# anulum/scpn-fusion-core

Measured on NVIDIA B200. Metric: converged_equilibria_per_s, higher is better.
Workload: dtype f64

## Files before the change

### scpn_fusion_core_b200/csrc/gsb_picard.cu

```cuda
#include "gsb_internal.cuh"
#include "gsb_resident.cuh"

#include <algorithm>
#include <cstdlib>

constexpr int kPT = 32;
constexpr int kTW = 8;
constexpr int kRW = 4;
constexpr int kSadChunk = 4096;
constexpr int kSadChunksMax = 64;

struct PicardState {
  int *active, *status, *iter, *cur, *best, *nxt, *xsel, *seed_active;
  double *diff_best, *gs_best, *gs_last, *diff_last, *scale;
  double *axbnd;
  double *topo;
};

struct Bufs {
  double *p[3];
};

struct gsb_picard_ws {
  int cap = 0;
// ... 957 lines not shown
  if (ir >= nr || iz >= nz) return;
  const size_t n = (size_t)nz * nr;
  double gz, gr;
  grad_point(psi + b * n, nz, nr, iz, ir, gg, gz, gr);
  const double rs = fmax(rrow[ir], 1e-6);
  const double inv = __ddiv_rn(1.0, rs);
  br[b * n + (size_t)iz * nr + ir] = dmul(-inv, gz);
  bz[b * n + (size_t)iz * nr + ir] = dmul(inv, gr);
}


struct PicardResArgs {
  double *psi;
  const double *bc;
  const double *ip;
  const double *prof_dev;
  double *jphi;
  double *summary;
  double *hist, *gs_hist;
  double *ws_psi;
  double *ws_src;
  const double *seedJ, *cf, *mr, *rrow;
  const int *rowmask;
  double seed_sum_drdz;
  int batch, max_iter, seed, saddle, need_gs, external;
  double tol, gs_tol, alpha, oma, omega;
  double dr, dz, dr2, dz2, four_drdz;
  GradGeom gg;
  ProfileDev prof;
  int scratch_off;
  int tplane_off;
  const int *order;
  const int *n_order;
};

__device__ __forceinline__ double pl(int xo, int nz, int hw, int iz, int ir) {
  return res_pool[xo + split_index(nz, hw, iz, ir)];
}

__device__ __forceinline__ void grad_planes(int xo, int nz, int nr, int hw, int iz, int ir, const GradGeom &gg,
                                            double &gz, double &gr) {
  const double c = pl(xo, nz, hw, iz, ir);
  if (iz == 0)
    gz = ddiv_y(dsub(pl(xo, nz, hw, 1, ir), c), gg.dz, gg.inv_dz);
  else if (iz == nz - 1)
    gz = ddiv_y(dsub(c, pl(xo, nz, hw, iz - 1, ir)), gg.dz, gg.inv_dz);
  else
    gz = ddiv_y(dsub(pl(xo, nz, hw, iz + 1, ir), pl(xo, nz, hw, iz - 1, ir)), gg.two_dz, gg.inv_two_dz);
  if (ir == 0)
    gr = ddiv_y(dsub(pl(xo, nz, hw, iz, 1), c), gg.dr, gg.inv_dr);
  else if (ir == nr - 1)
    gr = ddiv_y(dsub(c, pl(xo, nz, hw, iz, ir - 1)), gg.dr, gg.inv_dr);
  else
    gr = ddiv_y(dsub(pl(xo, nz, hw, iz, ir + 1), pl(xo, nz, hw, iz, ir - 1)), gg.two_dr, gg.inv_two_dr);
}

__device__ __forceinline__ double grad_mag(const GradGeom &gg, double c, double up, double down, double left,
                                           double right, bool z_lo, bool z_hi, bool r_lo, bool r_hi) {
  double gz, gr;
  if (z_lo)
    gz = ddiv_yf(dsub(up, c), gg.dz, gg.inv_dz);
  else if (z_hi)
    gz = ddiv_yf(dsub(c, down), gg.dz, gg.inv_dz);
  else
    gz = ddiv_yf(dsub(up, down), gg.two_dz, gg.inv_two_dz);
  if (r_lo)
// ... 11 lines not shown
  MtanhK mkp, mkf;
};
__device__ __forceinline__ double jraw_point(const JrawK &K, double v, double r, double cfv) {
  const double pn = ddiv_yf(dsub(v, K.psi_ax), K.denom, K.inv_denom);
  double pr = 0.0, ff = 0.0;
  if (pn >= 0.0 && pn < 1.0) {
    if (K.hmode) {
      pr = mtanh_res(pn, K.mkp);
      ff = K.same_prof ? pr : mtanh_res(pn, K.mkf);
    } else {
      pr = ff = dsub(1.0, pn);
    }
  }
  return dadd(dmul(0.5, dmul(r, pr)), dmul(0.5, dmul(cfv, ff)));
}

__device__ __forceinline__ double bcast_d(double v, int slot_off) {
  __syncthreads();
  if (threadIdx.x == 0) res_pool[slot_off] = v;
  __syncthreads();
  return res_pool[slot_off];
}

__global__ void __launch_bounds__(kResThreads, 1)
k_picard_resident(const __grid_constant__ RPlan plan, const __grid_constant__ PicardResArgs a) {
  const int lev_off = res_stage(plan);
  int nz, nr, hw, xo, f_lk, f_nch, f_rpc, f_nk;
  ResK rk;
  {
    const RLevel &F = res_level(lev_off, 0);
    nz = F.nz, nr = F.nr, hw = F.hw, xo = F.x_off, f_lk = F.lk, f_nch = F.nch, f_rpc = F.rpc, f_nk = F.nk;
    rk = res_load_resk(F.g);
  }
  const double *tab_ae = plan.lev[0].g.a_e;
  const double *tab_rs = plan.lev[0].g.r_safe, *tab_irs = plan.lev[0].g.inv_r_safe;
  const double a_ns0 = plan.lev[0].g.a_ns, a_c0 = plan.lev[0].g.a_c, inv_a_c0 = plan.lev[0].g.inv_a_c;
  const int n = nz * nr, ps = nz * hw, planes = 2 * ps, nslot = ps;
  const int tid = threadIdx.x, T = blockDim.x;
  const int lane = tid & 31, warp = tid >> 5, nw = T >> 5;
  const int step_z = T / hw, step_k = T - step_z * hw;
  const int iz_first = tid / hw, k_first = tid - iz_first * hw;
  double *sh = res_pool + a.scratch_off;
  int *shi = reinterpret_cast<int *>(sh + 32);
  const int bslot = a.scratch_off + 48;
  double *wpsi = a.ws_psi + (size_t)blockIdx.x * 3 * planes;
  double *wsrc = a.ws_src + (size_t)blockIdx.x * planes;
  const double n_all = (double)n, n_int = (double)(nz - 2) * (double)(nr - 2);
  const bool odd_nr = (nr & 1) != 0;

#define GSB_SLOT_LOOP_BEGIN()                                                  \
  for (int e = tid, iz = iz_first, k = k_first; e < nslot; e += T) {          \
    const int par_ = iz & 1;                                                   \
    const int pa = par_ * ps + e, pb = (1 - par_) * ps + e;                    \
    const bool has_odd = odd_nr ? (k < hw - 1) : true;
#define GSB_SLOT_LOOP_END()                                                    \
    k += step_k;                                                               \
    iz += step_z;                                                              \
    if (k >= hw) {                                                             \
      k -= hw;                                                                 \
      ++iz;                                                                    \
    }                                                                          \
  }

  const int n_work = a.order ? min(*a.n_order, a.batch) : a.batch;
  for (int wi = blockIdx.x; wi < n_work; wi += gridDim.x) {
    const int b = a.order ? a.order[wi] : wi;
    const double *bc = a.bc + (size_t)b * n;
    const double ipb = a.ip[b];
    double pp[4], pf[4];
#pragma unroll
    for (int i = 0; i < 4; ++i) {
      pp[i] = a.prof_dev ? a.prof_dev[(size_t)b * 8 + i] : a.prof.p[i];
      pf[i] = a.prof_dev ? a.prof_dev[(size_t)b * 8 + 4 + i] : a.prof.f[i];
    }
    const MtanhK mkp = mtanh_k(pp), mkf = mtanh_k(pf);
    const bool same_prof = pp[0] == pf[0] && pp[1] == pf[1] && pp[2] == pf[2] && pp[3] == pf[3];
    __syncthreads();
    res_load_dense(a.psi + (size_t)b * n, xo, nz, nr, hw);
    int cur = 0, best = 0, nxt = 1;
    const bool do_seed = a.seed && fabs(ipb) >= 1e-12;
    const double seed_sc = a.seed_sum_drdz > 0.0 ? __ddiv_rn(ipb, a.seed_sum_drdz) : 1.0;
    __syncthreads();
    if (a.seed) {
      for (int i = tid; i < planes; i += T) wpsi[2 * planes + i] = res_pool[xo + i];
      best = 2;
    }

    if (do_seed) {
      const double sc = seed_sc;
      for (int iz = warp; iz < nz; iz += nw)
        for (int ir = lane; ir < nr; ir += 32) {
          const double j = dmul(a.seedJ[iz * nr + ir], sc);
          wsrc[split_index(nz, hw, iz, ir)] = dmul(a.mr[ir], j);
        }
      __syncthreads();
      int p0 = xo, p1 = xo + ps, pt = a.tplane_off;
      for (int step = 0; step < 50; ++step) {
#pragma unroll 1
        for (int c = 0; c < 2; ++c) {
          const int src_plane = c == 0 ? p0 : p1;
          const int oth_plane = c == 0 ? p1 : p0;
          const int dst_plane = c == 0 ? pt : p1;
          int o = tid, iz = iz_first, k = k_first;
          while (o < nslot) {
            int vo[4], vz[4], vk[4];
            double vf[4];
#pragma unroll
            for (int u = 0; u < 4; ++u) {
              vo[u] = o, vz[u] = iz, vk[u] = k;
              const int s = (c + iz) & 1;
              const int ir = 2 * k + s;
              const bool interior = o < nslot && ir < nr && iz > 0 && iz < nz - 1 && ir > 0 && ir < nr - 1;
              vf[u] = interior ? __ldcg(wsrc + c * ps + o) : 0.0;
              o += T, k += step_k, iz += step_z;
              if (k >= hw) k -= hw, ++iz;
            }
#pragma unroll
            for (int u = 0; u < 4; ++u) {
              const int oo = vo[u], zz = vz[u];
              const int s = (c + zz) & 1;
              const int ir = 2 * vk[u] + s;
              if (oo < nslot && ir < nr) {
                double v;
                if (zz == 0 || zz == nz - 1 || ir == 0 || ir == nr - 1) {
                  v = sanitize_fast(res_pool[src_plane + oo]);
                } else {
                  const double cc = sanitize_fast(res_pool[oth_plane + oo]);
                  const double side = sanitize_fast(res_pool[oth_plane + oo - 1 + 2 * s]);
                  const double S = sanitize_fast(res_pool[oth_plane + oo - hw]), N = sanitize_fast(res_pool[oth_plane + oo + hw]);
                  const double f = sanitize_fast(vf[u]);
                  double acc = dadd(dmul(__ldg(tab_ae + ir), s ? side : cc), dmul(__ldg(tab_ae + nr + ir), s ? cc : side));
                  acc = dadd(acc, dmul(a_ns0, S));
                  acc = dadd(acc, dmul(a_ns0, N));
                  acc = dsub(acc, f);
                  v = clip_cap(ddiv_y(acc, a_c0, inv_a_c0));
                }
                res_pool[dst_plane + oo] = v;
              }
            }
          }
          __syncthreads();
        }
        const int t = p0;
        p0 = pt;
        pt = t;
      }
    }
    if (a.external && !do_seed) {
      for (int i = tid; i < planes; i += T) wsrc[i] = 0.0;
    }
    __syncthreads();
    for (int i = tid; i < planes; i += T) wpsi[(size_t)cur * planes + i] = res_pool[xo + i];
    __syncthreads();

    int status = 0, iters = 0;
    int j_slot = -1;
    bool j_ok = false;
    double diff_best = 1e9, gs_best = INFINITY, gs_last = INFINITY, diff_last = 0.0, scale = 0.0;
    double psi_ax = 0.0, psi_b = 0.0, t_izax = 0, t_irax = 0, t_izx = 0, t_irx = 0, t_found = 0;

    for (int kit = 0; kit < a.max_iter; ++kit) {
      GSB_PHASE_BEGIN();
      ValIdx mx{0.0, -1}, mb{0.0, -1};
      double mn = INFINITY;
      GSB_SLOT_LOOP_BEGIN()
        const int flat = iz * nr + 2 * k;
        const double ve = res_pool[xo + pa];
        const double vo = has_odd ? res_pool[xo + pb] : ve;
        if (ve > mx.v || mx.i < 0) mx = ValIdx{ve, flat};
        mn = fmin(mn, ve);
        if (has_odd) {
          if (vo > mx.v) mx = ValIdx{vo, flat + 1};
          mn = fmin(mn, vo);
        }
        if (__ldg(a.rowmask + iz) != 0) {
          const bool z_lo = iz == 0, z_hi = iz == nz - 1;
          {
            const double up = z_hi ? 0.0 : res_pool[xo + pb + hw], down = z_lo ? 0.0 : res_pool[xo + pb - hw];
            const double left = k > 0 ? res_pool[xo + pb - 1] : 0.0;
            const double bm = grad_mag(a.gg, ve, up, down, left, vo, z_lo, z_hi, k == 0, !has_odd);
            if (isfinite(bm)) mb = better<false>(mb, ValIdx{bm, flat});
          }
          if (has_odd) {
            const bool r_hi = 2 * k + 1 == nr - 1;
            const double up = z_hi ? 0.0 : res_pool[xo + pa + hw], down = z_lo ? 0.0 : res_pool[xo + pa - hw];
            const double right = r_hi ? 0.0 : res_pool[xo + pa + 1];
// ... 287 lines not shown
        res_pool[bslot] = code;
        res_pool[bslot + 1] = dbest;
        res_pool[bslot + 2] = gbest;
        res_pool[bslot + 3] = dl;
        res_pool[bslot + 4] = gl;
        res_pool[bslot + 5] = improved;
      }
      __syncthreads();
      const int code = (int)res_pool[bslot];
      diff_best = res_pool[bslot + 1];
      gs_best = res_pool[bslot + 2];
      diff_last = res_pool[bslot + 3];
      gs_last = res_pool[bslot + 4];
      const bool improved = res_pool[bslot + 5] != 0.0;
      __syncthreads();
      iters = kit + 1;
      GSB_PHASE(52);
      if (blockIdx.x == 0 && threadIdx.x == 0) GSB_PHASE_COUNT(53);
      if (code == 3) {
        status = 3;
        cur = best;
        break;
      }
      const int newcur = nxt;
      if (improved) best = newcur;
      cur = newcur;
      nxt = (cur == best) ? (cur == 0 ? 1 : 0) : 3 - cur - best;
      if (code != 0) {
        status = code;
        break;
      }
    }

    {
      const double *fin = wpsi + (size_t)cur * planes;
      const double *jsrc = wpsi + (size_t)(j_slot >= 0 ? j_slot : 0) * planes;
      JrawK jk;
      jk.psi_ax = psi_ax;
      jk.denom = dsub(psi_b, psi_ax);
      if (fabs(jk.denom) < 1e-9) jk.denom = 1e-9;
      jk.inv_denom = __ddiv_rn(1.0, jk.denom);
      jk.hmode = a.prof.hmode != 0, jk.same_prof = same_prof, jk.mkp = mkp, jk.mkf = mkf;
      double *po = a.psi + (size_t)b * n;
      double *jo = a.jphi + (size_t)b * n;
      for (int iz = warp; iz < nz; iz += nw)
        for (int ir = lane; ir < nr; ir += 32) {
          const int o = split_index(nz, hw, iz, ir);
          po[iz * nr + ir] = fin[o];
          double j;
          if (j_slot >= 0)
            j = j_ok ? dmul(jraw_point(jk, __ldcg(jsrc + o), __ldg(a.rrow + ir), __ldg(a.cf + ir)), scale) : 0.0;
          else
            j = do_seed ? dmul(a.seedJ[iz * nr + ir], seed_sc) : 0.0;
          jo[iz * nr + ir] = j;
        }
      if (threadIdx.x == 0 && a.summary) {
        double *o = a.summary + (size_t)b * 16;
        o[0] = (double)iters;
        o[1] = status == 1 ? 1.0 : 0.0;
        o[2] = diff_best;
        o[3] = gs_last;
        o[4] = gs_best;
        o[5] = (double)status;
        o[6] = psi_ax;
        o[7] = psi_b;
        o[8] = t_izax;
        o[9] = t_irax;
        o[10] = t_izx;
        o[11] = t_irx;
        o[12] = diff_last;
        o[13] = t_found;
        o[14] = scale;
        o[15] = 0.0;
      }
    }
    __syncthreads();
  }
#undef GSB_SLOT_LOOP_BEGIN
#undef GSB_SLOT_LOOP_END
}

__global__ void k_fb_init(int *__restrict__ mask, int *__restrict__ order, int *__restrict__ n_order,
                          double *__restrict__ fbsum, int batch) {
  const int b = blockIdx.x * blockDim.x + threadIdx.x;
  if (b == 0) *n_order = batch;
  if (b >= batch) return;
  mask[b] = 1;
  order[b] = b;
  fbsum[4 * b] = 0.0;
  fbsum[4 * b + 1] = INFINITY;
  fbsum[4 * b + 2] = 0.0;
  fbsum[4 * b + 3] = 0.0;
}

__device__ __forceinline__ int wall_index(int nz, int nr, int iz, int ir) {
  if (iz == 0) return ir;
  if (iz == nz - 1) return nr + 2 * (nz - 2) + ir;
  return nr + 2 * (iz - 1) + (ir ? 1 : 0);
}

__global__ void __launch_bounds__(256)
k_fb_prepare(double *__restrict__ psi, const double *__restrict__ ext, const double *__restrict__ wall,
             double *__restrict__ old, size_t n, int nz, int nr, int nwall, const int *__restrict__ mask) {
  const int b = blockIdx.y;
  if (!mask[b]) return;
  double *f = psi + (size_t)b * n;
  const double *e = ext + (size_t)b * n;
  double *o = old + (size_t)b * n;
// ... 628 lines not shown
  }
  if (!w->cand || w->cand_chunks < nchunks) {
    if (w->cand) cudaFree(w->cand);
    w->cand = nullptr;
    GSB_CUDA(cudaMalloc(&w->cand, (size_t)w->cap * nchunks * 32 * sizeof(double)));
    w->cand_chunks = nchunks;
  }
  k_saddle_cand<<<dim3(nchunks, batch), 256, 0, st>>>(bufs, cur, ctx->n, ctx->nz, ctx->nr, gg, w->mrows, w->n_mrows, nchunks, w->cand, active);
  GSB_LAUNCH_CHECK();
  k_saddle_pick<<<batch, 256, 0, st>>>(bufs, cur, ctx->n, ctx->nz, ctx->nr, dr2, dz2, four_drdz, nchunks, w->cand, xsel, active);
  GSB_LAUNCH_CHECK();
  return GSB_OK;
}

namespace gsb {
int picard_phase_read(long long *out64, int reset) {
#ifdef GSB_PHASE_TIMING
  long long tmp[64];
  GSB_CUDA(cudaMemcpyFromSymbol(tmp, g_phase, sizeof(tmp)));
  if (out64)
    for (int i = 0; i < 64; ++i) out64[i] += tmp[i];
  if (reset) {
    long long z[64] = {0};
    GSB_CUDA(cudaMemcpyToSymbol(g_phase, z, sizeof(z)));
  }
#else
  (void)out64;
  (void)reset;
#endif
  return GSB_OK;
}
}

static int picard_resident_launch(gsb_ctx *ctx, const gsb_picard_params *p, double *psi_dev, const double *bc_dev,
                                  const double *ip_dev, const double *prof_dev, double *jphi_dev,
                                  double *summary_dev, double *hist_dev, double *gs_hist_dev, int batch,
                                  const int *order_dev, const int *n_order_dev, cudaStream_t st) {
  constexpr int kScratch = 96;
  RPlan plan;
  if (!build_rplan(ctx, 0, kScratch, &plan) || plan.nlev < 2) return GSB_ESTATE;
  const int nz = ctx->nz, nr = ctx->nr, hw = (nr + 1) / 2;
  const RLevel &c1 = plan.lev[1];
  if (4 * c1.nz * c1.hw < nz * hw) return GSB_ESTATE;
  gsb_picard_ws *w = ctx->picard;
  const size_t planes = (size_t)2 * nz * hw, per_cta = 4 * planes;
  const int grid = std::min(batch, ctx->num_sms);
  if (w->res_grid < grid) {
    if (w->res_ws) cudaFree(w->res_ws);
    w->res_ws = nullptr;
    w->res_grid = 0;
    GSB_CUDA(cudaMalloc(&w->res_ws, (size_t)ctx->num_sms * per_cta * sizeof(double)));
    w->res_grid = ctx->num_sms;
  }
  PicardResArgs a{};
  a.psi = psi_dev;
  a.bc = bc_dev;
  a.ip = ip_dev;
  a.prof_dev = prof_dev;
  a.jphi = jphi_dev;
  a.summary = summary_dev;
  a.hist = hist_dev;
  a.gs_hist = gs_hist_dev;
  a.ws_psi = w->res_ws;
  a.ws_src = w->res_ws + (size_t)w->res_grid * 3 * planes;
  a.seedJ = w->seedJ;
  a.cf = w->cf;
  a.mr = w->mr;
  a.rrow = ctx->r_dev;
  a.rowmask = w->rowmask;
  {
    volatile double ssum = w->seed_sum * ctx->dr;
    volatile double ssum2 = ssum * ctx->dz;
    a.seed_sum_drdz = ssum2;
  }
  a.batch = batch;
  a.max_iter = p->max_iterations;
  a.seed = p->seed;
  a.saddle = p->saddle;
  a.need_gs = p->require_gs_residual;
  a.external = p->external_profile;
  a.tol = p->tol;
  a.gs_tol = p->gs_tol;
  a.alpha = p->alpha;
  a.oma = 1.0 - p->alpha;
  a.omega = p->omega;
  a.dr = ctx->dr;
  a.dz = ctx->dz;
  {
    volatile double dr2 = ctx->dr * ctx->dr, dz2 = ctx->dz * ctx->dz, f1 = 4.0 * ctx->dr, f2 = f1 * ctx->dz;
    a.dr2 = dr2;
    a.dz2 = dz2;
    a.four_drdz = f2;
  }
  a.gg = make_grad_geom(ctx->dz, ctx->dr);
  a.prof = to_dev(p->prof);
  a.scratch_off = plan.pool_doubles + res_stage_doubles(plan.nlev);
  a.tplane_off = c1.x_off;
  a.order = order_dev;
  a.n_order = n_order_dev;
  GSB_SMEM_OPT_IN(k_picard_resident, kResSmemMax);
  const size_t smem = (size_t)(a.scratch_off + kScratch) * sizeof(double);
  k_picard_resident<<<grid, kResThreads, smem, st>>>(plan, a);
  GSB_LAUNCH_CHECK();
  ctx->picard_last_iters = p->max_iterations;
  return GSB_OK;
}

extern "C" {

void gsb_picard_ws_free(gsb_ctx *ctx) {
  gsb_picard_ws *w = ctx->picard;
  if (!w) return;
  void *ptrs[] = {w->buf1, w->buf2, w->W, w->source, w->ring, w->tpart, w->spart, w->rpart,
                  w->seedJ, w->cf, w->mr, w->rowmask, w->ints, w->dbls, w->res_ws, w->mrows, w->cand,
                  w->and_psi, w->and_res, w->and_part, w->and_alpha, w->and_fb};
  for (void *q : ptrs)
    if (q) cudaFree(q);
  delete w;
  ctx->picard = nullptr;
}

int gsb_topology(gsb_ctx *ctx, const double *psi_dev, int batch, double z_min, int saddle,
                 double *out_dev, void *stream) {
  GSB_REQUIRE(ctx && psi_dev && out_dev, "gsb_topology: NULL argument");
  GSB_REQUIRE(batch >= 1 && batch <= ctx->batch_cap, "gsb_topology: batch outside [1, batch_cap]");
  GSB_CUDA(cudaSetDevice(ctx->device));
  gsb_picard_params p{};
  p.mu0 = 1.0;
  p.z_min = z_min;
  p.r_min = ctx->r_row.front();
  p.r_max = ctx->r_row.back();
  if (ctx->picard) {
// ... 37 lines not shown
    p.r_min = ctx->picard->r_min;
    p.r_max = ctx->picard->r_max;
  }
  int rc = picard_ws_ensure(ctx, &p);
  if (rc) return rc;
  gsb_picard_ws *w = ctx->picard;
  cudaStream_t st = (cudaStream_t)stream;
  Bufs bufs{{const_cast<double *>(psi_dev), nullptr, nullptr}};
  const int P = partials_for(ctx->nz, ctx->nr);
  k_source_raw<<<dim3(P, batch), 256, 0, st>>>(bufs, nullptr, ctx->n, ctx->nz, ctx->nr, axis_bnd_dev, to_dev(*prof),
                                               prof_dev, ctx->r_dev, w->cf, jphi_dev, w->spart, nullptr);
  GSB_LAUNCH_CHECK();
  k_source_scale<<<dim3(P, batch), 256, 0, st>>>(ctx->n, ctx->nz, ctx->nr, ctx->dr, ctx->dz, ip_dev, w->spart, P, w->mr,
                                                 jphi_dev, nullptr, nullptr, nullptr);
  GSB_LAUNCH_CHECK();
  return GSB_OK;
}

int gsb_b_field(gsb_ctx *ctx, const double *psi_dev, double *br_dev, double *bz_dev, int batch, void *stream) {
  GSB_REQUIRE(ctx && psi_dev && br_dev && bz_dev, "gsb_b_field: NULL argument");
  GSB_REQUIRE(batch >= 1 && batch <= 65535, "gsb_b_field: bad batch");
  GSB_CUDA(cudaSetDevice(ctx->device));
  const dim3 blk(32, 8, 1), grd((ctx->nr + 31) / 32, (ctx->nz + 7) / 8, batch);
  k_bfield<<<grd, blk, 0, (cudaStream_t)stream>>>(psi_dev, ctx->nz, ctx->nr, make_grad_geom(ctx->dz, ctx->dr), ctx->r_dev, br_dev, bz_dev);
  GSB_LAUNCH_CHECK();
  return GSB_OK;
}

int gsb_picard_last_launched_iterations(gsb_ctx *ctx) { return ctx ? ctx->picard_last_iters : 0; }

static int picard_solve_impl(gsb_ctx *ctx, const gsb_picard_params *p, double *psi_dev, const double *bc_dev,
                             const double *ip_dev, const double *prof_dev, double *jphi_dev, double *summary_dev,
                             double *hist_dev, double *gs_hist_dev, int batch, const int *mask_dev,
                             const int *order_dev, const int *n_order_dev, void *stream) {
  GSB_REQUIRE(ctx && p && psi_dev && bc_dev && ip_dev && jphi_dev && summary_dev, "gsb_picard_solve: NULL argument");
  GSB_REQUIRE(batch >= 1 && batch <= ctx->batch_cap, "gsb_picard_solve: batch outside [1, batch_cap]");
  GSB_REQUIRE(p->max_iterations >= 1, "gsb_picard_solve: max_iterations must be >= 1");
  GSB_REQUIRE(p->method >= 0 && p->method <= 3, "gsb_picard_solve: unknown method");
  GSB_REQUIRE(p->method != 3 || (p->anderson_depth >= 0 && p->anderson_depth <= kAndMax),
              "gsb_picard_solve: anderson_depth outside [0, 8]");
  GSB_REQUIRE(std::isfinite(p->omega) && p->omega >= 1.0 && p->omega < 2.0,
              "omega must be finite and satisfy 1.0 <= omega < 2.0");
  GSB_REQUIRE(!p->require_gs_residual || p->gs_tol > 0.0, "solver.gs_residual_threshold must be > 0");
  GSB_CUDA(cudaSetDevice(ctx->device));
  int rc = ensure_plan(ctx, 5);
  if (rc) return rc;
  rc = picard_ws_ensure(ctx, p);
  if (rc) return rc;
  gsb_picard_ws *w = ctx->picard;
  cudaStream_t st = (cudaStream_t)stream;
  const int nz = ctx->nz, nr = ctx->nr;
  const size_t n = ctx->n;
  const LevelGeom &g = ctx->levels[0].g;
  Bufs bufs{{psi_dev, w->buf1, w->buf2}};
  PicardState &s = w->s;
  const int P = partials_for(nz, nr);
  const GradGeom gg = make_grad_geom(ctx->dz, ctx->dr);
  if (p->method == 0 && !std::getenv("GSB_PICARD_STREAMING")) {
    rc = picard_resident_launch(ctx, p, psi_dev, bc_dev, ip_dev, prof_dev, jphi_dev, summary_dev, hist_dev,
                                gs_hist_dev, batch, order_dev, n_order_dev, st);
    if (rc != GSB_ESTATE) return rc;
  }
  const int copy_blocks = (int)std::min<size_t>((n + 255) / 256, 64);
  const ProfileDev prof = to_dev(p->prof);

  const bool use_graph = !std::getenv("GSB_NO_GRAPH");
  cudaStream_t caller = st;
  if (use_graph) {
    if (!ctx->gstream) {
      GSB_CUDA(cudaStreamCreateWithFlags(&ctx->gstream, cudaStreamNonBlocking));
      GSB_CUDA(cudaEventCreateWithFlags(&ctx->gevent, cudaEventDisableTiming));
    }
    GSB_CUDA(cudaEventRecord(ctx->gevent, caller));
    GSB_CUDA(cudaStreamWaitEvent(ctx->gstream, ctx->gevent, 0));
    st = ctx->gstream;
  }

  k_picard_init<<<(batch + 127) / 128, 128, 0, st>>>(s, batch, p->seed ? 2 : 0, ip_dev, p->seed, mask_dev);
  GSB_LAUNCH_CHECK();
  rc = ring_save_launch(bc_dev, n, w->ring, nz, nr, batch, st);
  if (rc) return rc;
  if (p->external_profile) {
    GSB_REQUIRE(mask_dev == nullptr, "external_profile_mode is not combined with a masked (free-boundary batch) solve");
    GSB_CUDA(cudaMemsetAsync(jphi_dev, 0, (size_t)batch * n * sizeof(double), st));
    GSB_CUDA(cudaMemsetAsync(w->source, 0, (size_t)batch * n * sizeof(double), st));
  }
  if (p->seed) {
    GSB_CUDA(cudaMemcpyAsync(w->buf2, psi_dev, (size_t)batch * n * sizeof(double), cudaMemcpyDeviceToDevice, st));
    volatile double ssum = w->seed_sum * ctx->dr;
    volatile double ssum2 = ssum * ctx->dz;
    k_seed_source<<<dim3(copy_blocks, batch), 256, 0, st>>>(n, nr, w->seedJ, ssum2, ip_dev, w->mr, jphi_dev, w->source, s.seed_active);
    GSB_LAUNCH_CHECK();
    rc = jacobi_steps_launch(ctx, psi_dev, w->W, w->source, 50, batch, s.seed_active, st);
    if (rc) return rc;
  }
// ... 152 lines not shown
int gsb_picard_solve(gsb_ctx *ctx, const gsb_picard_params *p, double *psi_dev, const double *bc_dev,
                     const double *ip_dev, const double *prof_dev, double *jphi_dev, double *summary_dev,
                     double *hist_dev, double *gs_hist_dev, int batch, void *stream) {
  return picard_solve_impl(ctx, p, psi_dev, bc_dev, ip_dev, prof_dev, jphi_dev, summary_dev, hist_dev, gs_hist_dev,
                           batch, nullptr, nullptr, nullptr, stream);
}

struct ShapeStep {
  ShapeFitArgs fit;
  const double *wts;
  const int *corner;
  const double *target;
  const double *green;
};

static int free_boundary_loop(gsb_ctx *ctx, const gsb_picard_params *p, const gsb_free_boundary_params *fb,
                              const ShapeStep *sh, double *psi_dev, double *psi_ext_dev, const double *wall_m_dev,
                              const double *ip_dev, const double *prof_dev, double *jphi_dev, double *summary_dev,
                              double *fb_summary_dev, int batch, void *stream) {
  GSB_CUDA(cudaSetDevice(ctx->device));
  cudaStream_t st = (cudaStream_t)stream;
  const size_t n = ctx->n;
  const int nz = ctx->nz, nr = ctx->nr, nw = ctx->n_wall;
  const size_t cap = (size_t)ctx->batch_cap;
  if (!ctx->fb_old) GSB_CUDA(cudaMalloc(&ctx->fb_old, cap * n * sizeof(double)));
  if (!ctx->fb_part) GSB_CUDA(cudaMalloc(&ctx->fb_part, cap * kPT * 2 * sizeof(double)));
  if (!ctx->fb_ints) GSB_CUDA(cudaMalloc(&ctx->fb_ints, (2 * cap + 2) * sizeof(int)));
  if (wall_m_dev && !ctx->fb_wall) GSB_CUDA(cudaMalloc(&ctx->fb_wall, cap * nw * sizeof(double)));
  double *old = ctx->fb_old, *part = ctx->fb_part, *wall = wall_m_dev ? ctx->fb_wall : nullptr;
  int *mask = ctx->fb_ints, *order = ctx->fb_ints + batch, *n_order = ctx->fb_ints + 2 * batch;
  const int P = partials_for(nz, nr);
  const int blocks = (int)std::min<size_t>((n + 255) / 256, 64);
  int rc = GSB_OK;
  k_fb_init<<<(batch + 255) / 256, 256, 0, st>>>(mask, order, n_order, fb_summary_dev, batch);
  GSB_LAUNCH_CHECK();
  const double dA = ctx->dr * ctx->dz;
  cudaEvent_t ev[4] = {nullptr, nullptr, nullptr, nullptr};
  if (ctx->timing)
    for (auto &e : ev) GSB_CUDA(cudaEventCreate(&e));
  int outer = 0;
  for (; outer < fb->max_outer_iter; ++outer) {
    const bool with_wall = wall_m_dev && (outer > 0 || fb->warm_j);
    if (with_wall) {
      if (ctx->timing) cudaEventRecord(ev[2], st);
      rc = gsb_wall_flux(ctx, wall_m_dev, jphi_dev, dA, wall, batch, stream);
      if (rc) break;
      if (ctx->timing) cudaEventRecord(ev[3], st);
    }
    k_fb_prepare<<<dim3(blocks, batch), 256, 0, st>>>(psi_dev, psi_ext_dev, with_wall ? wall : nullptr, old, n, nz, nr, nw, mask);
    GSB_LAUNCH_CHECK();
    if (ctx->timing) cudaEventRecord(ev[0], st);
    rc = picard_solve_impl(ctx, p, psi_dev, psi_dev , ip_dev, prof_dev, jphi_dev,
                           summary_dev, nullptr, nullptr, batch, mask, order, n_order, stream);
    if (rc) break;
    if (ctx->timing) cudaEventRecord(ev[1], st);
    if (sh) {
      const int Pt = sh->fit.P;
      k_shape_target<<<batch, 256, 0, st>>>(psi_dev, n, nr, sh->wts, sh->corner, Pt, sh->target, sh->fit.out, mask);
      GSB_LAUNCH_CHECK();
      ShapeFitArgs a = sh->fit;
      a.mask = mask;
      k_shape_fit<<<(batch + kShapeWarps - 1) / kShapeWarps, 32 * kShapeWarps, 0, st>>>(a);
      GSB_LAUNCH_CHECK();
      rc = gsb_coil_flux(ctx, sh->green, a.w, a.n, 1, psi_ext_dev, batch, stream);
      if (rc) break;
    }
    k_fb_diff<<<dim3(P, batch), 256, 0, st>>>(psi_dev, old, n, part, mask);
    GSB_LAUNCH_CHECK();
    k_fb_decide<<<1, 1024, 0, st>>>(part, P, fb->tol, outer, summary_dev, fb_summary_dev, mask, order, n_order, batch);
    GSB_LAUNCH_CHECK();
    GSB_CUDA(cudaMemcpyAsync(ctx->h_counter, n_order, sizeof(int), cudaMemcpyDeviceToHost, st));
    GSB_CUDA(cudaStreamSynchronize(st));
// ... 230 lines not shown
```

### scpn_fusion_core_b200/csrc/gsb_resident.cuh

```cuda
#pragma once

#include "gsb_internal.cuh"

namespace gsb {

constexpr int kResThreads = 512;
constexpr int kResMaxLevels = 12;
constexpr int kResSmemMax = 232448;

struct RLevel {
  int nz, nr, hw, nk;
  int x_off;
  int d_off;
  int t_off;
  int lk;
  int nch, rpc;
  int lj;
  int cch, crpc;
  LevelGeom g;
};
struct RPlan {
  int nlev;
  int pool_doubles;
  RLevel lev[kResMaxLevels];
};
static_assert(sizeof(RLevel) % 8 == 0, "RLevel is staged to shared memory in 8-byte words");
inline int res_stage_doubles(int nlev) { return nlev * (int)(sizeof(RLevel) / 8); }

extern __shared__ double res_pool[];

__device__ __forceinline__ const RLevel &res_level(int lev_off, int l) {
  return reinterpret_cast<const RLevel *>(res_pool + lev_off)[l];
}

#ifdef GSB_PHASE_TIMING
__device__ long long g_phase[64];
#define GSB_PHASE_BEGIN() long long _pt = clock64()
#define GSB_PHASE(idx)                                      \
  do {                                                      \
    if (blockIdx.x == 0 && threadIdx.x == 0) {              \
      const long long _now = clock64();                     \
      g_phase[(idx)] += _now - _pt;                         \
      _pt = _now;                                           \
    }                                                       \
  } while (0)
#define GSB_PHASE_COUNT(idx) g_phase[(idx)] += 1
#else
#define GSB_PHASE_BEGIN() do {} while (0)
#define GSB_PHASE(idx) do {} while (0)
#define GSB_PHASE_COUNT(idx) do {} while (0)
#endif

__device__ __forceinline__ int split_index(int nz, int hw, int iz, int ir) {
  return (((iz + ir) & 1) * nz + iz) * hw + (ir >> 1);
}

__device__ __forceinline__ double ddiv_yf(double a, double b, double y) {
  const double q = __dmul_rn(a, y);
  const double r = __fma_rn(-b, q, a);
  return __fma_rn(r, y, q);
}

__device__ __forceinline__ void res_load_dense(const double *__restrict__ g, int xo, int nz, int nr,
                                               int hw) {
  const int lane = threadIdx.x & 31, warp = threadIdx.x >> 5, nw = blockDim.x >> 5;
  for (int iz = warp; iz < nz; iz += nw) {
    const double *row = g + (size_t)iz * nr;
    for (int ir = lane; ir < nr; ir += 32) res_pool[xo + (((iz + ir) & 1) * nz + iz) * hw + (ir >> 1)] = row[ir];
  }
}
__device__ __forceinline__ void res_store_dense(double *__restrict__ g, int xo, int nz, int nr, int hw) {
  const int lane = threadIdx.x & 31, warp = threadIdx.x >> 5, nw = blockDim.x >> 5;
  for (int iz = warp; iz < nz; iz += nw) {
    double *row = g + (size_t)iz * nr;
    for (int ir = lane; ir < nr; ir += 32) row[ir] = res_pool[xo + (((iz + ir) & 1) * nz + iz) * hw + (ir >> 1)];
  }
}

struct SorK {
  double a_ns, a_c, inv_a_c, omega, omw;
};

template <int S>
// ... 172 lines not shown
  if (GR) {
    double r[kResMaxRun];
    auto fetch = [&](int par) {
      const double *rg = rhs_g + par * ps + o;
#pragma unroll
      for (int t = 0; t < kResMaxRun; ++t) r[t] = (t < cnt) ? __ldcg(rg + t * hw) : 0.0;
    };
    if (active) fetch(first & 1);
    for (int pass = 0; pass < npass; ++pass) {
      if (active) {
        const int par = (first + pass) & 1;
        const int P = x_off + par * ps + o, Q = x_off + (1 - par) * ps + o;
        if ((par + z0) & 1)
          res_smooth_run_pref<1>(P, Q, hw, cnt, ae1, aw1, ok1, ae0, aw0, ok0, c, r);
        else
          res_smooth_run_pref<0>(P, Q, hw, cnt, ae0, aw0, ok0, ae1, aw1, ok1, c, r);
        if (pass + 1 < npass) fetch(1 - par);
      }
      __syncthreads();
    }
  } else {
    for (int pass = 0; pass < npass; ++pass) {
      if (active) {
        const int par = (first + pass) & 1;
        const int P = x_off + par * ps + o, Q = x_off + (1 - par) * ps + o;
        const int ro = d_off + par * ps + o;
        if ((par + z0) & 1)
          res_smooth_run<1>(P, Q, ro, hw, cnt, ae1, aw1, ok1, ae0, aw0, ok0, c);
        else
          res_smooth_run<0>(P, Q, ro, hw, cnt, ae0, aw0, ok0, ae1, aw1, ok1, c);
      }
      __syncthreads();
    }
  }
}

struct ResK {
  double dr2, dz2, two_dr, inv_dr2, inv_dz2, inv_two_dr;
};
__device__ __forceinline__ double res_lx(const ResK &g, double rs, double inv_rs, double C, double E, double W, double S,
                                         double N) {
  const double twoC = dmul(2.0, C);
  const double d2r = ddiv_yf(dadd(dsub(E, twoC), W), g.dr2, g.inv_dr2);
  const double d1r = ddiv_yf(dsub(E, W), g.two_dr, g.inv_two_dr);
  const double d2z = ddiv_yf(dadd(dsub(N, twoC), S), g.dz2, g.inv_dz2);
  return dadd(dsub(d2r, ddiv_yf(d1r, rs, inv_rs)), d2z);
}
__device__ __forceinline__ ResK res_load_resk(const LevelGeom &g) {
  ResK k;
  k.dr2 = g.dr2, k.dz2 = g.dz2, k.two_dr = g.two_dr, k.inv_dr2 = g.inv_dr2, k.inv_dz2 = g.inv_dz2,
  k.inv_two_dr = g.inv_two_dr;
  return k;
}

struct Row5 {
  double v0, v1, v2, v3, v4;
};
struct Row3 {
  double a, b, c;
};

template <bool GR>
__device__ __noinline__ void res_residual_restrict(int lev_off, int l, const double *__restrict__ rhs_g) {
  int nz, hw, xo, fd_off, cnz, cnr, chw, cd_off, lj, cch, crpc;
  ResK g;
  const double *ts, *ti;
// ... 253 lines not shown
```

Before: 4135.

## Fuse free-boundary outer loop into resident Picard kernel and restructure seed Jacobi

Moves the free-boundary outer iteration, with wall boundary reset, old-psi snapshot, max-difference convergence test and summary write, inside the resident Picard kernel. This replaces the host-driven loop of separate kernel launches when no shape or wall coupling is used. The seed Jacobi smoother is also rewritten as a column-run routine that keeps rows in registers and prefetches the RHS, replacing the strided slot loop. The cost is an extra per-CTA workspace plane and more device-side control flow.

```diff
diff --git a/scpn_fusion_core_b200/csrc/gsb_picard.cu b/scpn_fusion_core_b200/csrc/gsb_picard.cu
--- a/scpn_fusion_core_b200/csrc/gsb_picard.cu
+++ b/scpn_fusion_core_b200/csrc/gsb_picard.cu
@@ -1013,6 +1013,10 @@
   int tplane_off;
   const int *order;
   const int *n_order;
+  double *ws_old;
+  double *fb_summary;
+  int max_outer;
+  double fb_tol;
 };
 
 __device__ __forceinline__ double pl(int xo, int nz, int hw, int iz, int ir) {
@@ -1090,9 +1094,7 @@
     nz = F.nz, nr = F.nr, hw = F.hw, xo = F.x_off, f_lk = F.lk, f_nch = F.nch, f_rpc = F.rpc, f_nk = F.nk;
     rk = res_load_resk(F.g);
   }
-  const double *tab_ae = plan.lev[0].g.a_e;
   const double *tab_rs = plan.lev[0].g.r_safe, *tab_irs = plan.lev[0].g.inv_r_safe;
-  const double a_ns0 = plan.lev[0].g.a_ns, a_c0 = plan.lev[0].g.a_c, inv_a_c0 = plan.lev[0].g.inv_a_c;
   const int n = nz * nr, ps = nz * hw, planes = 2 * ps, nslot = ps;
   const int tid = threadIdx.x, T = blockDim.x;
   const int lane = tid & 31, warp = tid >> 5, nw = T >> 5;
@@ -1135,6 +1137,20 @@
     const bool same_prof = pp[0] == pf[0] && pp[1] == pf[1] && pp[2] == pf[2] && pp[3] == pf[3];
     __syncthreads();
     res_load_dense(a.psi + (size_t)b * n, xo, nz, nr, hw);
+    if (threadIdx.x == 0) res_pool[bslot + 16] = 0.0, res_pool[bslot + 17] = 0.0;
+    for (;;) {
+    GSB_PHASE_BEGIN();
+    if (a.max_outer > 0) {
+      __syncthreads();
+      for (int i = tid; i < 2 * nr + 2 * (nz - 2); i += T) {
+        int iz, ir;
+        res_wall_point(i, nz, nr, iz, ir);
+        res_pool[xo + split_index(nz, hw, iz, ir)] = bc[iz * nr + ir];
+      }
+      __syncthreads();
+      double *wold = a.ws_old + (size_t)blockIdx.x * planes;
+      for (int i = tid; i < planes; i += T) wold[i] = res_pool[xo + i];
+    }
     int cur = 0, best = 0, nxt = 1;
     const bool do_seed = a.seed && fabs(ipb) >= 1e-12;
     const double seed_sc = a.seed_sum_drdz > 0.0 ? __ddiv_rn(ipb, a.seed_sum_drdz) : 1.0;
@@ -1144,6 +1160,7 @@
       best = 2;
     }
 
+    GSB_PHASE(55);
     if (do_seed) {
       const double sc = seed_sc;
       for (int iz = warp; iz < nz; iz += nw)
@@ -1152,64 +1169,16 @@
           wsrc[split_index(nz, hw, iz, ir)] = dmul(a.mr[ir], j);
         }
       __syncthreads();
-      int p0 = xo, p1 = xo + ps, pt = a.tplane_off;
-      for (int step = 0; step < 50; ++step) {
-#pragma unroll 1
-        for (int c = 0; c < 2; ++c) {
-          const int src_plane = c == 0 ? p0 : p1;
-          const int oth_plane = c == 0 ? p1 : p0;
-          const int dst_plane = c == 0 ? pt : p1;
-          int o = tid, iz = iz_first, k = k_first;
-          while (o < nslot) {
-            int vo[4], vz[4], vk[4];
-            double vf[4];
-#pragma unroll
-            for (int u = 0; u < 4; ++u) {
-              vo[u] = o, vz[u] = iz, vk[u] = k;
-              const int s = (c + iz) & 1;
-              const int ir = 2 * k + s;
-              const bool interior = o < nslot && ir < nr && iz > 0 && iz < nz - 1 && ir > 0 && ir < nr - 1;
-              vf[u] = interior ? __ldcg(wsrc + c * ps + o) : 0.0;
-              o += T, k += step_k, iz += step_z;
-              if (k >= hw) k -= hw, ++iz;
-            }
-#pragma unroll
-            for (int u = 0; u < 4; ++u) {
-              const int oo = vo[u], zz = vz[u];
-              const int s = (c + zz) & 1;
-              const int ir = 2 * vk[u] + s;
-              if (oo < nslot && ir < nr) {
-                double v;
-                if (zz == 0 || zz == nz - 1 || ir == 0 || ir == nr - 1) {
-                  v = sanitize_fast(res_pool[src_plane + oo]);
-                } else {
-                  const double cc = sanitize_fast(res_pool[oth_plane + oo]);
-                  const double side = sanitize_fast(res_pool[oth_plane + oo - 1 + 2 * s]);
-                  const double S = sanitize_fast(res_pool[oth_plane + oo - hw]), N = sanitize_fast(res_pool[oth_plane + oo + hw]);
-                  const double f = sanitize_fast(vf[u]);
-                  double acc = dadd(dmul(__ldg(tab_ae + ir), s ? side : cc), dmul(__ldg(tab_ae + nr + ir), s ? cc : side));
-                  acc = dadd(acc, dmul(a_ns0, S));
-                  acc = dadd(acc, dmul(a_ns0, N));
-                  acc = dsub(acc, f);
-                  v = clip_cap(ddiv_y(acc, a_c0, inv_a_c0));
-                }
-                res_pool[dst_plane + oo] = v;
-              }
-            }
-          }
-          __syncthreads();
-        }
-        const int t = p0;
-        p0 = pt;
-        pt = t;
-      }
+      res_jacobi_seed(lev_off, wsrc, a.tplane_off, 50);
     }
     if (a.external && !do_seed) {
       for (int i = tid; i < planes; i += T) wsrc[i] = 0.0;
     }
+    GSB_PHASE(54);
     __syncthreads();
     for (int i = tid; i < planes; i += T) wpsi[(size_t)cur * planes + i] = res_pool[xo + i];
     __syncthreads();
+    GSB_PHASE(55);
 
     int status = 0, iters = 0;
     int j_slot = -1;
@@ -1563,6 +1532,51 @@
       }
     }
 
+    GSB_PHASE_RESTART();
+    if (a.max_outer > 0) {
+      if (status == 3) {
+        const double *fin = wpsi + (size_t)cur * planes;
+        for (int i = tid; i < planes; i += T) res_pool[xo + i] = __ldcg(fin + i);
+        __syncthreads();
+      }
+      const double *wold = a.ws_old + (size_t)blockIdx.x * planes;
+      double m = 0.0;
+      int bad = 0;
+      GSB_SLOT_LOOP_BEGIN()
+        const double de = fabs(dsub(res_pool[xo + pa], __ldcg(wold + pa)));
+        if (de != de) bad = 1;
+        m = fmax(m, de);
+        if (has_odd) {
+          const double dd = fabs(dsub(res_pool[xo + pb], __ldcg(wold + pb)));
+          if (dd != dd) bad = 1;
+          m = fmax(m, dd);
+        }
+      GSB_SLOT_LOOP_END()
+      const int anybad = __syncthreads_or(bad);
+      m = block_max(m, sh);
+      if (threadIdx.x == 0) {
+        const double diff = anybad ? NAN : m;
+        const double outer = res_pool[bslot + 16] + 1.0;
+        const double it_sum = res_pool[bslot + 17] + (double)iters;
+        const bool conv = diff < a.fb_tol, done = conv || outer >= (double)a.max_outer;
+        res_pool[bslot + 16] = outer;
+        res_pool[bslot + 17] = it_sum;
+        res_pool[bslot + 18] = done ? 1.0 : 0.0;
+        if (done) {
+          double *f = a.fb_summary + (size_t)b * 4;
+          f[0] = outer;
+          f[1] = diff;
+          f[2] = it_sum;
+          f[3] = conv ? 1.0 : 0.0;
+        }
+      }
+      __syncthreads();
+      if (res_pool[bslot + 18] == 0.0) {
+        GSB_PHASE(55);
+        continue;
+      }
+    }
+
     {
       const double *fin = wpsi + (size_t)cur * planes;
       const double *jsrc = wpsi + (size_t)(j_slot >= 0 ? j_slot : 0) * planes;
@@ -1605,6 +1619,9 @@
         o[15] = 0.0;
       }
     }
+    GSB_PHASE(55);
+    break;
+    }
     __syncthreads();
   }
 #undef GSB_SLOT_LOOP_BEGIN
@@ -2299,10 +2316,16 @@
 }
 }
 
+struct FbOuter {
+  int max_outer;
+  double tol;
+  double *fb_summary;
+};
+
 static int picard_resident_launch(gsb_ctx *ctx, const gsb_picard_params *p, double *psi_dev, const double *bc_dev,
                                   const double *ip_dev, const double *prof_dev, double *jphi_dev,
                                   double *summary_dev, double *hist_dev, double *gs_hist_dev, int batch,
-                                  const int *order_dev, const int *n_order_dev, cudaStream_t st) {
+                                  const int *order_dev, const int *n_order_dev, const FbOuter *fo, cudaStream_t st) {
   constexpr int kScratch = 96;
   RPlan plan;
   if (!build_rplan(ctx, 0, kScratch, &plan) || plan.nlev < 2) return GSB_ESTATE;
@@ -2310,7 +2333,7 @@
   const RLevel &c1 = plan.lev[1];
   if (4 * c1.nz * c1.hw < nz * hw) return GSB_ESTATE;
   gsb_picard_ws *w = ctx->picard;
-  const size_t planes = (size_t)2 * nz * hw, per_cta = 4 * planes;
+  const size_t planes = (size_t)2 * nz * hw, per_cta = 5 * planes;
   const int grid = std::min(batch, ctx->num_sms);
   if (w->res_grid < grid) {
     if (w->res_ws) cudaFree(w->res_ws);
@@ -2330,6 +2353,7 @@
   a.gs_hist = gs_hist_dev;
   a.ws_psi = w->res_ws;
   a.ws_src = w->res_ws + (size_t)w->res_grid * 3 * planes;
+  a.ws_old = w->res_ws + (size_t)w->res_grid * 4 * planes;
   a.seedJ = w->seedJ;
   a.cf = w->cf;
   a.mr = w->mr;
@@ -2365,6 +2389,11 @@
   a.tplane_off = c1.x_off;
   a.order = order_dev;
   a.n_order = n_order_dev;
+  if (fo) {
+    a.max_outer = fo->max_outer;
+    a.fb_tol = fo->tol;
+    a.fb_summary = fo->fb_summary;
+  }
   GSB_SMEM_OPT_IN(k_picard_resident, kResSmemMax);
   const size_t smem = (size_t)(a.scratch_off + kScratch) * sizeof(double);
   k_picard_resident<<<grid, kResThreads, smem, st>>>(plan, a);
@@ -2468,7 +2497,7 @@
 static int picard_solve_impl(gsb_ctx *ctx, const gsb_picard_params *p, double *psi_dev, const double *bc_dev,
                              const double *ip_dev, const double *prof_dev, double *jphi_dev, double *summary_dev,
                              double *hist_dev, double *gs_hist_dev, int batch, const int *mask_dev,
-                             const int *order_dev, const int *n_order_dev, void *stream) {
+                             const int *order_dev, const int *n_order_dev, void *stream, const FbOuter *fo = nullptr) {
   GSB_REQUIRE(ctx && p && psi_dev && bc_dev && ip_dev && jphi_dev && summary_dev, "gsb_picard_solve: NULL argument");
   GSB_REQUIRE(batch >= 1 && batch <= ctx->batch_cap, "gsb_picard_solve: batch outside [1, batch_cap]");
   GSB_REQUIRE(p->max_iterations >= 1, "gsb_picard_solve: max_iterations must be >= 1");
@@ -2494,9 +2523,10 @@
   const GradGeom gg = make_grad_geom(ctx->dz, ctx->dr);
   if (p->method == 0 && !std::getenv("GSB_PICARD_STREAMING")) {
     rc = picard_resident_launch(ctx, p, psi_dev, bc_dev, ip_dev, prof_dev, jphi_dev, summary_dev, hist_dev,
-                                gs_hist_dev, batch, order_dev, n_order_dev, st);
+                                gs_hist_dev, batch, order_dev, n_order_dev, fo, st);
     if (rc != GSB_ESTATE) return rc;
   }
+  if (fo) return GSB_ESTATE;
   const int copy_blocks = (int)std::min<size_t>((n + 255) / 256, 64);
   const ProfileDev prof = to_dev(p->prof);
 
@@ -2715,12 +2745,30 @@
   const int P = partials_for(nz, nr);
   const int blocks = (int)std::min<size_t>((n + 255) / 256, 64);
   int rc = GSB_OK;
+  cudaEvent_t ev[4] = {nullptr, nullptr, nullptr, nullptr};
+  if (ctx->timing)
+    for (auto &e : ev) GSB_CUDA(cudaEventCreate(&e));
+  if (!sh && !wall_m_dev) {
+    const FbOuter fo{fb->max_outer_iter, fb->tol, fb_summary_dev};
+    if (ctx->timing) cudaEventRecord(ev[0], st);
+    rc = picard_solve_impl(ctx, p, psi_dev, psi_ext_dev, ip_dev, prof_dev, jphi_dev, summary_dev, nullptr, nullptr, batch,
+                           nullptr, nullptr, nullptr, stream, &fo);
+    if (rc != GSB_ESTATE) {
+      if (rc == GSB_OK && ctx->timing) {
+        float ms = 0.f;
+        cudaEventRecord(ev[1], st);
+        if (cudaEventSynchronize(ev[1]) == cudaSuccess && cudaEventElapsedTime(&ms, ev[0], ev[1]) == cudaSuccess)
+          ctx->timing_acc[0] += ms, ctx->timing_acc[1] += 1.0;
+      }
+      for (auto &e : ev)
+        if (e) cudaEventDestroy(e);
+      return rc;
+    }
+    rc = GSB_OK;
+  }
   k_fb_init<<<(batch + 255) / 256, 256, 0, st>>>(mask, order, n_order, fb_summary_dev, batch);
   GSB_LAUNCH_CHECK();
   const double dA = ctx->dr * ctx->dz;
-  cudaEvent_t ev[4] = {nullptr, nullptr, nullptr, nullptr};
-  if (ctx->timing)
-    for (auto &e : ev) GSB_CUDA(cudaEventCreate(&e));
   int outer = 0;
   for (; outer < fb->max_outer_iter; ++outer) {
     const bool with_wall = wall_m_dev && (outer > 0 || fb->warm_j);
diff --git a/scpn_fusion_core_b200/csrc/gsb_resident.cuh b/scpn_fusion_core_b200/csrc/gsb_resident.cuh
--- a/scpn_fusion_core_b200/csrc/gsb_resident.cuh
+++ b/scpn_fusion_core_b200/csrc/gsb_resident.cuh
@@ -45,10 +45,12 @@
     }                                                       \
   } while (0)
 #define GSB_PHASE_COUNT(idx) g_phase[(idx)] += 1
+#define GSB_PHASE_RESTART() _pt = clock64()
 #else
 #define GSB_PHASE_BEGIN() do {} while (0)
 #define GSB_PHASE(idx) do {} while (0)
 #define GSB_PHASE_COUNT(idx) do {} while (0)
+#define GSB_PHASE_RESTART() do {} while (0)
 #endif
 
 __device__ __forceinline__ int split_index(int nz, int hw, int iz, int ir) {
@@ -287,6 +289,141 @@
       }
       __syncthreads();
     }
+  }
+}
+
+__device__ __forceinline__ void res_wall_point(int i, int nz, int nr, int &iz, int &ir) {
+  if (i < nr) {
+    iz = 0, ir = i;
+  } else if (i < nr + 2 * (nz - 2)) {
+    iz = 1 + ((i - nr) >> 1), ir = ((i - nr) & 1) ? nr - 1 : 0;
+  } else {
+    iz = nz - 1, ir = i - nr - 2 * (nz - 2);
+  }
+}
+
+struct JacK {
+  double ae0, aw0, ae1, aw1, a_ns, a_c, inv_a_c;
+};
+template <int S>
+__device__ __forceinline__ double res_jacobi_update(const JacK &j, double side, double c_prev, double c_cur,
+                                                    double c_next, double f) {
+  double acc = dadd(dmul(S ? j.ae1 : j.ae0, S ? side : c_cur), dmul(S ? j.aw1 : j.aw0, S ? c_cur : side));
+  acc = dadd(acc, dmul(j.a_ns, c_prev));
+  acc = dadd(acc, dmul(j.a_ns, c_next));
+  acc = dsub(acc, f);
+  return clip_cap(ddiv_y(acc, j.a_c, j.inv_a_c));
+}
+
+template <int S0>
+__device__ __forceinline__ void res_jacobi_run_pref(int po, int qo, int hw, int cnt, const JacK &j, bool ok0, bool ok1,
+                                                    const double *__restrict__ rg) {
+  double r[kResMaxRun];
+#pragma unroll
+  for (int t = 0; t < kResMaxRun; ++t) r[t] = (t < cnt) ? __ldcg(rg + t * hw) : 0.0;
+  constexpr int dA = S0 ? 1 : -1, dB = S0 ? -1 : 1;
+  const bool okA = S0 ? ok1 : ok0, okB = S0 ? ok0 : ok1;
+  double c_prev = sanitize_fast(res_pool[qo - hw]), c_cur = sanitize_fast(res_pool[qo]);
+#pragma unroll
+  for (int g = 0; g < kResMaxRun / 4; ++g) {
+    if (4 * g + 4 <= cnt) {
+      const int q1 = qo + hw, q2 = q1 + hw, q3 = q2 + hw, q4 = q3 + hw;
+      const int p1 = po + hw, p2 = p1 + hw, p3 = p2 + hw;
+      const double c1 = sanitize_fast(res_pool[q1]), c2 = sanitize_fast(res_pool[q2]);
+      const double c3 = sanitize_fast(res_pool[q3]), c4 = sanitize_fast(res_pool[q4]);
+      const double s0 = sanitize_fast(res_pool[qo + dA]), s1 = sanitize_fast(res_pool[q1 + dB]);
+      const double s2 = sanitize_fast(res_pool[q2 + dA]), s3 = sanitize_fast(res_pool[q3 + dB]);
+      const double v0 = res_jacobi_update<S0>(j, s0, c_prev, c_cur, c1, sanitize_fast(r[4 * g]));
+      const double v1 = res_jacobi_update<1 - S0>(j, s1, c_cur, c1, c2, sanitize_fast(r[4 * g + 1]));
+      const double v2 = res_jacobi_update<S0>(j, s2, c1, c2, c3, sanitize_fast(r[4 * g + 2]));
+      const double v3 = res_jacobi_update<1 - S0>(j, s3, c2, c3, c4, sanitize_fast(r[4 * g + 3]));
+      if (okA) {
+        res_pool[po] = v0;
+        res_pool[p2] = v2;
+      }
+      if (okB) {
+        res_pool[p1] = v1;
+        res_pool[p3] = v3;
+      }
+      c_prev = c3;
+      c_cur = c4;
+      po = p3 + hw;
+      qo = q4;
+    } else if (4 * g < cnt) {
+#pragma unroll
+      for (int t = 0; t < 3; ++t) {
+        if (4 * g + t < cnt) {
+          const double c1 = sanitize_fast(res_pool[qo + hw]);
+          const double f = sanitize_fast(r[4 * g + t]);
+          if ((t & 1) == 0) {
+            const double v = res_jacobi_update<S0>(j, sanitize_fast(res_pool[qo + dA]), c_prev, c_cur, c1, f);
+            if (okA) res_pool[po] = v;
+          } else {
+            const double v = res_jacobi_update<1 - S0>(j, sanitize_fast(res_pool[qo + dB]), c_prev, c_cur, c1, f);
+            if (okB) res_pool[po] = v;
+          }
+          c_prev = c_cur;
+          c_cur = c1;
+          po += hw;
+          qo += hw;
+        }
+      }
+    }
+  }
+}
+
+static __device__ __noinline__ void res_jacobi_seed(int lev_off, const double *__restrict__ rhs_g, int t_plane, int steps) {
+  int nz, nr, hw, nk, x_off, lk, nch, rpc;
+  JacK j;
+  const double *tab;
+  {
+    const RLevel &L = res_level(lev_off, 0);
+    nz = L.nz, nr = L.nr, hw = L.hw, nk = L.nk, x_off = L.x_off, lk = L.lk, nch = L.nch, rpc = L.rpc;
+    j.a_ns = L.g.a_ns, j.a_c = L.g.a_c, j.inv_a_c = L.g.inv_a_c;
+    tab = L.g.a_e;
+  }
+  const int ps = nz * hw, T = blockDim.x, tid = threadIdx.x;
+  for (int i = tid; i < 2 * nr + 2 * (nz - 2); i += T) {
+    int iz, ir;
+    res_wall_point(i, nz, nr, iz, ir);
+    const int o = split_index(nz, hw, iz, ir);
+    const double v = sanitize_fast(res_pool[x_off + o]);
+    res_pool[x_off + o] = v;
+    if (o < ps) res_pool[t_plane + o] = v;
+  }
+  const int k = tid & ((1 << lk) - 1), ch = tid >> lk;
+  const int z0 = 1 + ch * rpc;
+  const int z1 = min(z0 + rpc, nz - 1);
+  const bool active = (ch < nch) && (k < nk) && (z0 < z1);
+  const int ir0 = 2 * k, ir1 = 2 * k + 1;
+  j.ae0 = j.aw0 = j.ae1 = j.aw1 = 0.0;
+  if (active) {
+    j.ae0 = __ldg(tab + ir0);
+    j.aw0 = __ldg(tab + nr + ir0);
+    if (ir1 < nr) {
+      j.ae1 = __ldg(tab + ir1);
+      j.aw1 = __ldg(tab + nr + ir1);
+    }
+  }
+  const bool ok0 = ir0 >= 1 && ir0 <= nr - 2, ok1 = ir1 <= nr - 2;
+  const int o = z0 * hw + k, cnt = z1 - z0;
+  __syncthreads();
+  int p0 = x_off, p1 = x_off + ps, pt = t_plane;
+  for (int step = 0; step < steps; ++step) {
+#pragma unroll 1
+    for (int c = 0; c < 2; ++c) {
+      if (active) {
+        const int P = (c == 0 ? pt : p1) + o, Q = (c == 0 ? p1 : p0) + o;
+        if ((c + z0) & 1)
+          res_jacobi_run_pref<1>(P, Q, hw, cnt, j, ok0, ok1, rhs_g + c * ps + o);
+        else
+          res_jacobi_run_pref<0>(P, Q, hw, cnt, j, ok0, ok1, rhs_g + c * ps + o);
+      }
+      __syncthreads();
+    }
+    const int t = p0;
+    p0 = pt;
+    pt = t;
   }
 }
 
```

New measurement: 4146, median of 6. No clear change (+0.3%).
